# spaceml-org/STARCOP

Measured on AMD Instinct MI355X. Metric: 512x512 hyperspectral tiles/sec (train fwd+bwd), higher is better.
Workload: dtype f32; 1 GPU; configs[1]: HyperSTARCOP U-Net (smp.Unet mobilenet_v2, 4ch mag1c+RGB) train step fwd+loss+bwd+Adam, 512x512 tiles, fp32 HIP kernels (3x3 convs: fp32 operands split exactly into 16-bit terms on the matrix cores, fp32 accumulation; see config.precision and DESIGN.md section 2); batch_per_gpu=16, global_batch=16, parallelism=dp1, hipgraph=False, precision=fp32

## Files before the change

include/starcop_hip.h:

```cpp
#ifndef STARCOP_HIP_H
#define STARCOP_HIP_H

#include <stddef.h>
#include <stdint.h>

#ifdef __cplusplus
extern "C" {
#endif

typedef void* sc_stream;

enum sc_status {
  SC_OK = 0,
  SC_ERR_ARG = -1,
  SC_ERR_LAUNCH = -2,
  SC_ERR_NOTPD = -3,
  SC_ERR_NODEV = -4
};

enum sc_src_mode {
  SC_SRC_RAW = 0,
  SC_SRC_AFFINE = 1,
  SC_SRC_BNBWD = 2,
  SC_SRC_NORM = 3
// ... 69 lines not shown
size_t sc_packed_weight_floats_bx3(int Cout, int Cin, int co_t, int transpose_flip, int terms);
int sc_conv3x3_bx3(const sc_conv_args* a, sc_stream stream);

typedef struct sc_wgrad_args {
  sc_src dy;
  sc_src src[2];
  int32_t nsrc;
  int32_t N, H, W, Cout, Cin, ks;
  float* part; size_t part_floats;
  float* dw;
  int32_t terms;
  const float* absmax;
  const float* xbound[2];
} sc_wgrad_args;
size_t sc_wgrad_workspace_floats(int N, int H, int W, int Cout, int Cin, int ks);
int sc_conv2d_wgrad_mfma(const sc_wgrad_args* a, sc_stream stream);
typedef struct sc_wgrad_pending {
  const float* part; float* dw;
  int32_t nparts, taps, Cout, Cin, CoP, CiP;
  uint64_t total;
} sc_wgrad_pending;
int sc_conv2d_wgrad_mfma_deferred(const sc_wgrad_args* a, sc_wgrad_pending* pending_host, sc_stream stream);
int sc_wgrad_reduce_batch(const sc_wgrad_pending* descs_dev, const uint32_t* block_starts_dev, int n, uint32_t total_blocks,
                          sc_stream stream);
#define SC_PACK_THIN16 5
#define SC_PACK_PW3 6
size_t sc_packed_weight_floats_thin16(int Cout, int Cin, int transpose_flip);
int sc_pack_weights_thin16(const float* w_oihw, float* wpk, int Cout, int Cin, int transpose_flip, sc_stream stream);
int sc_conv3x3_thin16(const sc_conv_args* a, sc_stream stream);

#define SC_PACK_SP 7
size_t sc_packed_weight_floats_sp(int Cout, int Cup, int Cskip);
int sc_pack_weights_sp(const float* w_oihw, float* wpk, int Cout, int Cup, int Cskip, int terms, sc_stream stream);
int sc_sp_stat_rows(int N, int H, int W, int Cout);
int sc_conv3x3_sp(const sc_conv_args* a, sc_stream stream);
#define SC_PACK_SPD 8
size_t sc_packed_weight_floats_spd(int Cout, int Cup, int Cskip_tiles );
int sc_spd_vskip_ok(int Cup, int Cskip);
int sc_pack_weights_spd(const float* w_oihw, float* wpk, int Cout, int CinTotal, int Cup, int vskip, int terms, sc_stream stream);
int sc_conv3x3_sp_dgrad(const sc_conv_args* a, sc_stream stream);
size_t sc_sp_wgrad_workspace_bytes(int N, int H, int W, int Cout, int Cup);
int sc_conv3x3_sp_wgrad(const sc_wgrad_args* a, void* ws, size_t ws_bytes, sc_stream stream);
int sc_wgrad_scatter_cols(const float* src, float* dw, int Cout, int Ccols, int CinTotal, int col_off, sc_stream stream);

size_t sc_wgrad_thin16_workspace_floats(int N, int H, int W, int Cout, int Cin);
int sc_conv3x3_wgrad_thin16(const sc_wgrad_args* a, sc_stream stream);

size_t sc_packed_weight_floats_pw3(int Cout, int Cin, int transpose_flip);
int sc_conv1x1_pw3(const sc_conv_args* a, sc_stream stream);
int sc_conv1x1_pw3_variant(int N, int H, int W, int Cout);
size_t sc_wgrad_pw3_workspace_floats(int N, int H, int W, int Cout, int Cin);
int sc_conv1x1_wgrad_pw3(const sc_wgrad_args* a, sc_wgrad_pending* pending_host, sc_stream stream);
int sc_wgrad_pw3_variant(int N, int H, int W, int Cout, int Cin);

typedef struct sc_irb_args {
  sc_src x;
  const float* wpk_expand;
  const float* cst_expand;
  const float* w_dw;
  const float* cst_dw;
  const float* wpk_project;
  const float* cst_project;
  float* out;
  float* z_absmax;
  int32_t N, Cin, hidden, Cout, H, W, stride, residual;
} sc_irb_args;
int sc_irb_supported(int Cin, int hidden, int Cout, int H, int W, int stride);
int sc_irb_variant(int Cin, int hidden, int Cout, int stride);
int sc_irb_eval(const sc_irb_args* a, sc_stream stream);

typedef struct sc_irt_args {
  sc_src x;
  const float* w_expand;
  const float* w_dw;
  const float* cst_expand;
  int32_t N, Cin, hidden, H, W, stride;
} sc_irt_args;
int sc_irt_supported(int Cin, int hidden, int H, int W, int stride);
int sc_irt_rows(int stage, int N, int H, int W, int stride);
int sc_irt_bwd_rows(int N, int hidden, int H, int W);
size_t sc_irt_bwd_workspace_floats(int N, int Cin, int hidden, int H, int W);
int sc_irt_expand_stats(const sc_irt_args* a, float* stats , sc_stream stream);
int sc_irt_fwd(const sc_irt_args* a, float* d_out , float* stats_d , sc_stream stream);
int sc_irt_bwd(const sc_irt_args* a, const sc_src* dy_d, double* e_sums , double* dw_acc ,
               float* work, sc_stream stream);
int sc_irt_xmoments(const sc_irt_args* a, float* work, sc_stream stream);
int sc_irt_bwd_fix(const sc_irt_args* a, const float* cst_bwd_expand, float* work, float* dx, const float* add0, int accum,
                   sc_stream stream);
int sc_irt_wgrad_finalize(const sc_irt_args* a, const float* cst_bwd_expand, float* work, float* dw_expand, sc_stream stream);

size_t sc_wgrad_bx3_workspace_floats(int N, int H, int W, int Cout, int Cin);
int sc_conv3x3_wgrad_bx3(const sc_wgrad_args* a, sc_stream stream);

int sc_dwconv3x3_fwd(const sc_src* in, const float* w , float* out,
                     int N, int C, int Hin, int Win, int stride, float* stats ,
                     sc_stream stream);
typedef struct sc_bn_tail {
  const float* gamma; const float* beta;
  float* running_mean; float* running_var;
  float momentum, eps;
  float* cst;
  float* act_bound;
  uint32_t* tickets;
} sc_bn_tail;
int sc_dwconv3x3_fwd_bn(const sc_src* in, const float* w, float* out, int N, int C, int Hin, int Win, int stride, float* stats,
                        const sc_bn_tail* bn, sc_stream stream);
// ... 351 lines not shown
```

starcop_amd/_lib.py:

```python
import ctypes as C
import os
import subprocess

import torch

_HERE = os.path.dirname(os.path.abspath(__file__))
LIB_PATH = os.path.join(_HERE, "libstarcop_hip.so")
CSRC = os.path.join(_HERE, "csrc")

SC_CST = 8
STAT_CONV3, STAT_CONV1, STAT_DW, STAT_STEM, STAT_BNBWD, STAT_CONV1K, STAT_PW3 = 0, 1, 2, 3, 4, 5, 6

SRC_RAW, SRC_AFFINE, SRC_BNBWD, SRC_NORM = 0, 1, 2, 3
ACT_NONE, ACT_RELU, ACT_RELU6 = 0, 1, 2


class StarcopHipError(RuntimeError):
    pass


class sc_src(C.Structure):
    _fields_ = [("x", C.c_void_p), ("aux", C.c_void_p), ("cst", C.c_void_p),
                ("C", C.c_int32), ("mode", C.c_int32), ("act", C.c_int32), ("up", C.c_int32)]

# ... 210 lines not shown
    "sc_valid_mask_ne": (_i, [_vp, _i, _i, _i, _i, _d, C.c_int64, _vp, _vp]),
    "sc_mag1c_layout_columns": (_i, [_vp, _i, _i, _vp, _i, _i, _i, _vp, _vp, _vp, _vp, _vp, _vp, _vp]),
    "sc_mag1c_layout_ids_workspace_ints": (_sz, [C.c_int64, _i]),
    "sc_mag1c_layout_ids": (_i, [_vp, _vp, C.c_int64, _i, _i, _i, _vp, _vp, _vp, _vp, _vp, _vp, _vp, _vp]),
    "sc_trimmed_sum_workspace_bytes": (_sz, [_i]),
    "sc_trimmed_sums": (_i, [_vp, _i, _sz, _d, _vp, _vp, _sz, _vp]),
    "sc_band_ratio": (_i, [_vp, _vp, _vp, _i, _sz, _vp, _vp, _f, _f, _vp]),
    "sc_clip_scale": (_i, [_vp, _vp, _sz, _f, _f, _f, _f, _i, _vp]),
    "sc_mlr_workspace_bytes": (_sz, [_i, _sz, _i]),
    "sc_mlr_moments": (_i, [C.POINTER(sc_mlr_args), _vp, _sz, _vp]),
    "sc_mlr_solve": (_i, [C.POINTER(sc_mlr_args), _vp, _vp, _sz, _vp]),
    "sc_mlr_fit": (_i, [C.POINTER(sc_mlr_args), _vp, _vp, _sz, _vp]),
    "sc_mlr_predict": (_i, [C.POINTER(sc_mlr_args), _vp, _vp, _vp]),
    "sc_mlr_ratio": (_i, [C.POINTER(sc_mlr_args), _vp, _vp, _i, _i, _vp, _vp, _sz, _vp]),
    "sc_label_workspace_bytes": (_sz, [_i, _i, _i]),
    "sc_srf_bands": (_i, [C.POINTER(sc_srf_args), _vp]),
    "sc_window_stats_workspace_bytes": (_sz, [_i]),
    "sc_window_stats": (_i, [C.POINTER(sc_winstats_args), _vp, _sz, _vp]),
    "sc_glt_ortho": (_i, [C.POINTER(sc_ortho_args), _vp]),
    "sc_window_cut": (_i, [C.POINTER(sc_wcut_args), _vp]),
    "sc_scene_gather": (_i, [C.POINTER(sc_scene_args), _vp]),
    "sc_head_conv_fwd_k_mosaic": (_i, [C.POINTER(sc_src), _vp, _vp, _vp, _i, _i, C.c_int64, _vp, _vp, _i, _i, _i, _i, _i, _vp]),
    "sc_connected_components": (_i, [_vp, _i, _vp, _vp, _vp, _sz, _i, _i, _i, _vp]),
    "sc_proposed_mask": (_i, [_vp, C.c_int64, _vp, C.c_int64, _f, _i, _vp, _vp, _sz, _i, _i, _i, _vp]),
    "sc_packed_weight_floats_thin16": (_sz, [_i, _i, _i]),
    "sc_pack_weights_thin16": (_i, [_vp, _vp, _i, _i, _i, _vp]),
    "sc_conv3x3_thin16": (_i, [C.POINTER(sc_conv_args), _vp]),
    "sc_packed_weight_floats_sp": (_sz, [_i, _i, _i]),
    "sc_pack_weights_sp": (_i, [_vp, _vp, _i, _i, _i, _i, _vp]),
    "sc_sp_stat_rows": (_i, [_i, _i, _i, _i]),
    "sc_conv3x3_sp": (_i, [C.POINTER(sc_conv_args), _vp]),
    "sc_packed_weight_floats_spd": (_sz, [_i, _i, _i]),
    "sc_pack_weights_spd": (_i, [_vp, _vp, _i, _i, _i, _i, _i, _vp]),
    "sc_spd_vskip_ok": (_i, [_i, _i]),
    "sc_conv3x3_sp_dgrad": (_i, [C.POINTER(sc_conv_args), _vp]),
    "sc_sp_wgrad_workspace_bytes": (_sz, [_i, _i, _i, _i, _i]),
    "sc_conv3x3_sp_wgrad": (_i, [C.POINTER(sc_wgrad_args), _vp, _sz, _vp]),
    "sc_wgrad_scatter_cols": (_i, [_vp, _vp, _i, _i, _i, _i, _vp]),
    "sc_binary_opening": (_i, [_vp, _f, _i, _vp, _vp, _i, _i, _i, _vp]),
    "sc_threshold_confusion": (_i, [_vp, _vp, _vp, _vp, _i, _i, _vp, _vp, _i, _i, _i, _vp]),
    "sc_gather_augment": (_i, [_vp, _i, _i, _i, _i, _vp, _vp, _vp, _vp, _vp, _vp, _i, _i, _i, _i, _vp, _vp]),
    "sc_tile_window_sums": (_i, [_vp, _i, _i, _i, _vp, _vp, _i, _vp, _vp]),
    "sc_dwconv3x3_bwd_fused": (_i, [C.POINTER(sc_src), C.POINTER(sc_src), _vp, _vp, _vp, _vp, _i, _i, _i, _i, _i, _vp]),
    "sc_wgrad_thin16_workspace_floats": (_sz, [_i, _i, _i, _i, _i]),
    "sc_conv3x3_wgrad_thin16": (_i, [C.POINTER(sc_wgrad_args), _vp]),
    "sc_conv2d_wgrad_mfma_deferred": (_i, [C.POINTER(sc_wgrad_args), C.POINTER(sc_wgrad_pending), _vp]),
    "sc_wgrad_reduce_batch": (_i, [_vp, _vp, _i, C.c_uint32, _vp]),
    "sc_packed_weight_floats_pw3": (_sz, [_i, _i, _i]),
    "sc_conv1x1_pw3": (_i, [C.POINTER(sc_conv_args), _vp]),
    "sc_conv1x1_pw3_variant": (_i, [_i, _i, _i, _i]),
    "sc_wgrad_pw3_workspace_floats": (_sz, [_i, _i, _i, _i, _i]),
    "sc_wgrad_pw3_variant": (_i, [_i, _i, _i, _i, _i]),
    "sc_conv1x1_wgrad_pw3": (_i, [C.POINTER(sc_wgrad_args), C.POINTER(sc_wgrad_pending), _vp]),
    "sc_irb_supported": (_i, [_i, _i, _i, _i, _i, _i]),
    "sc_irb_variant": (_i, [_i, _i, _i, _i]),
    "sc_irb_eval": (_i, [C.POINTER(sc_irb_args), _vp]),
    "sc_irt_supported": (_i, [_i, _i, _i, _i, _i]),
    "sc_irt_rows": (_i, [_i, _i, _i, _i, _i]),
    "sc_irt_bwd_rows": (_i, [_i, _i, _i, _i]),
    "sc_irt_bwd_workspace_floats": (_sz, [_i, _i, _i, _i, _i]),
    "sc_irt_expand_stats": (_i, [C.POINTER(sc_irt_args), _vp, _vp]),
    "sc_irt_fwd": (_i, [C.POINTER(sc_irt_args), _vp, _vp, _vp]),
    "sc_irt_bwd": (_i, [C.POINTER(sc_irt_args), C.POINTER(sc_src), _vp, _vp, _vp, _vp]),
    "sc_irt_xmoments": (_i, [C.POINTER(sc_irt_args), _vp, _vp]),
    "sc_irt_bwd_fix": (_i, [C.POINTER(sc_irt_args), _vp, _vp, _vp, _vp, _i, _vp]),
    "sc_irt_wgrad_finalize": (_i, [C.POINTER(sc_irt_args), _vp, _vp, _vp, _vp]),
    "sc_maxpool2x2": (_i, [C.POINTER(sc_src), _vp, _i, _i, _i, _i, _vp]),
    "sc_upsample_bilinear2x": (_i, [C.POINTER(sc_src), _vp, _i, _i, _i, _i, _vp]),
    "sc_maxpool2x2_bwd": (_i, [C.POINTER(sc_src), _vp, _vp, _i, _i, _i, _i, _i, _vp]),
    "sc_upsample_bilinear2x_bwd": (_i, [_vp, _vp, _i, _i, _i, _i, _vp]),
    "sc_pwreg_param_floats": (_sz, [_i, _i, _i, _i]),
    "sc_pwreg_fwd": (_i, [_vp, _vp, _i, _i, _i, _i, _i, _i, _i, _vp, _vp]),
    "sc_reg_loss": (_i, [_vp, _vp, _sz, _i, _vp, _vp, _vp, _vp]),
    "sc_pwreg_sweep_blocks": (_i, [_i, _i, _i]),
    "sc_pwreg_train_sweep": (_i, [_vp, _vp, _vp, _i, _i, _i, _i, _i, _i, _i, _i, _vp, _vp]),
    "sc_pwreg_finalize": (_i, [_vp, _i, _vp, _i, _i, _i, _i, _d, _vp, _vp, _vp]),
    "sc_panel_minmax": (_i, [_vp, C.POINTER(sc_panel), _i, _vp, _vp]),
    "sc_render_panels": (_i, [_vp, C.POINTER(sc_panel), _i, _vp, _vp, _i, _i, _vp]),
    "sc_component_stats_workspace_bytes": (_sz, [_i, _i, _i, _i, _i]),
    "sc_component_stats": (_i, [C.POINTER(sc_cstats_args), _vp, _sz, _vp]),
    "sc_tiff_lzw_decode": (_i, [_vp, _sz, _vp, _sz, C.POINTER(C.c_size_t)]),
    "sc_tiff_unpredict": (_i, [_vp, _i, _i, _i, _i, _i, _i, _vp]),
}
REG_L1, REG_MSE, PWREG_G_FROM_MEMORY = 0, 1, 2
PWREG_MAXC, PWREG_PART_DOUBLES, REG_LOSS_PARTS = 16, 273, 256
PACK_SPD = 8
PACK_SP = 7
PACK_PW3 = 6
PACK_THIN16 = 5
TERMS_F16X2 = 4
SE_CROSS = 0xBA

_lib = None


def build(force=False):
    if force:
        subprocess.run(["make", "-C", CSRC, "clean"], check=True, stdout=subprocess.DEVNULL)
    r = subprocess.run(["make", "-C", CSRC, "-j", "4"], capture_output=True, text=True)
    if r.returncode != 0:
        raise StarcopHipError("building libstarcop_hip.so failed:\n" + r.stdout[-4000:] + r.stderr[-4000:])
    return LIB_PATH


def load():
    global _lib
# ... 76 lines not shown
```

starcop_amd/network.py:

```python
import ctypes as C
import math
import os

import torch
import torch.nn as nn

from . import _lib
from ._lib import (ACT_NONE, ACT_RELU, ACT_RELU6, SC_CST, sc_irb_args, sc_irt_args, SRC_AFFINE, SRC_BNBWD, SRC_NORM, SRC_RAW, STAT_BNBWD, sc_wgrad_pending,
                   PACK_PW3, PACK_SP, PACK_SPD, PACK_THIN16, STAT_PW3, STAT_CONV1, STAT_CONV1K, STAT_CONV3, STAT_DW, STAT_STEM, TERMS_F16X2, check, make_src, ptr, sc_bn_tail, sc_bnr_args,
                   sc_conv_args, sc_wgrad_args, stream)

MBV2_SETTINGS = ((1, 16, 1, 1), (6, 24, 2, 2), (6, 32, 3, 2), (6, 64, 4, 2),
                 (6, 96, 3, 1), (6, 160, 3, 2), (6, 320, 1, 1))
DECODER_CHANNELS = (256, 128, 64, 32, 16)
BN_EPS, BN_MOMENTUM = 1e-5, 0.1


def _conv_bn_act(cin, cout, k, stride=1, groups=1, act="relu6"):
    return nn.Sequential(nn.Conv2d(cin, cout, k, stride, (k - 1) // 2, groups=groups, bias=False),
                         nn.BatchNorm2d(cout, eps=BN_EPS, momentum=BN_MOMENTUM),
                         nn.ReLU6() if act == "relu6" else nn.ReLU())


class _InvertedResidual(nn.Module):
# ... 38 lines not shown
        cskips = (96, 32, 24, 16, 0)
        self.blocks = nn.ModuleList(_DecoderBlock(i, s, o) for i, s, o in zip(cins, cskips, DECODER_CHANNELS))


class _T:
    __slots__ = ("name", "C", "shift", "kind", "bn", "act", "buf", "grad", "cst", "cstb", "stats", "bsums",
                 "grad_written", "alias_grad_of", "res_grad")

    def __init__(self, name, Cn, shift, kind, bn=None, act=ACT_NONE):
        self.name, self.C, self.shift, self.kind, self.bn, self.act = name, Cn, shift, kind, bn, act
        self.buf = self.grad = self.cst = self.cstb = self.stats = self.bsums = None
        self.grad_written = False
        self.alias_grad_of = None
        self.res_grad = None


_BN_PRE = True
_COT_RATIO = 1.15
_COT_RATIO3 = 1.15
_HEAD_FUSED_BWD = True


def _pick_cot(M, ks=1):
    if M <= 16 and ks == 3:
        return 16
    if M <= 32:
        return 32
    p32, p64 = -(-M // 32) * 32, -(-M // 64) * 64
    return 64 if p64 <= p32 * (_COT_RATIO3 if ks == 3 else _COT_RATIO) else 32


_PW3 = os.environ.get("STARCOP_PW3", "1")
_PWS64 = os.environ.get("STARCOP_PWS64", "1") == "1"


def _use_pw3(which, N, HW, Cin, Cout):
    if _PW3 == "0" or (which == 2 and HW % 8):
        return False
    if _PW3 == "all":
        return True
    NP = N * HW
    npb = -(-NP // 32)
    if _PWS64 and HW == 4096 and which in (0, 1):
        K_, M_ = (Cin, Cout) if which == 0 else (Cout, Cin)
        if K_ in (16, 24, 32) and M_ <= 192 and (which == 1 or K_ in (24, 32)):
            return False
    if which == 0:
        return HW <= 4096 and (Cin <= 320 or npb * (-(-Cout // 32)) >= 1024)
    if which == 1:
        K, MB = Cout, -(-Cin // 32)
        return (K <= 192 and HW <= 4096 and NP <= 131072) or (K > 192 and HW <= 1024 and npb * MB >= 2048)
    KM = Cin * Cout
    return HW <= 1024 and NP <= 32768 and KM <= 300000 and (HW <= 256 or KM <= 32768)


_IRT = os.environ.get("STARCOP_IRT", "1")


def _use_irt(N, Cin, Hd, Hin, Win, stride):
    if _IRT == "0" or not _lib.load().sc_irt_supported(Cin, Hd, Hin, Win, stride):
        return False
    return _IRT == "all" or (Hin * Win >= 65536 and 4 * N * Hd * Hin * Win >= (256 << 20))


_IRB = os.environ.get("STARCOP_IRB", "1")


def _use_irb(N, Cin, hidden, Cout, H, W, stride):
    if _IRB == "0" or not _lib.load().sc_irb_supported(Cin, hidden, Cout, H, W, stride):
        return False
    if _IRB == "all":
        return True
    if stride == 2:
        return Cin <= 64 and hidden % 64 == 0 and H * W <= 25600
    return Cin <= 96 and hidden % 64 == 0 and Cout <= 128 and H * W <= 6400


_SP = os.environ.get("STARCOP_SP", "1")
_BNR = os.environ.get("STARCOP_BNR", "0") == "1"
_BNR_THIN = os.environ.get("STARCOP_BNR_THIN", "0") == "1"
_THIN_SPD = os.environ.get("STARCOP_THIN_SPD", "1") == "1"
_PACK_SIDE = os.environ.get("STARCOP_PACK_SIDE", "1") == "1"
_DW_TAIL_ROWS = int(os.environ.get("STARCOP_DW_TAIL_ROWS", "0"))
_SP_SKIPTILES = os.environ.get("STARCOP_SP_SKIPTILES", "1") == "1"


def _experiment(name, default=""):
    v = os.environ.get(name, default)
    if v not in ("", "0"):
        if os.environ.get("STARCOP_EXPERIMENT_OK") != "1":
            raise RuntimeError(f"{name}={v} is an elimination experiment (wrong results by design); set STARCOP_EXPERIMENT_OK=1 to run it")
        import warnings
        warnings.warn(f"starcop_amd: elimination experiment {name}={v} is ACTIVE -- results of this process are wrong by design")
    return v


_EXP_NO_WGRAD = _experiment("STARCOP_EXP_NO_WGRAD", "0") == "1"
_EXP_NO_BNFIN = _experiment("STARCOP_EXP_NO_BNFIN", "")
_EXP_SIDE2 = _experiment("STARCOP_EXP_SIDE2", "0") == "1"


_SP_TERMS = (TERMS_F16X2, 1)


def _use_sp(N, Ho, Wo, Cout):
    if _SP == "0" or Ho % 2 or Wo % 2:
# ... 363 lines not shown
            n_dw = 0
            irt_e = {self._ops[i]["out"].name for i in plan.irt}
            plan.irt_esums, plan.irt_work = {}, {}
            for i_e in plan.irt:
                cv, tin, te = self._ops[i_e]["conv"], self._ops[i_e]["ins"][0], self._ops[i_e]["out"]
                Hi, Wi = H >> tin.shift, W >> tin.shift
                plan.irt_esums[te.name] = torch.empty(lib.sc_irt_bwd_rows(N, cv.out_channels, Hi, Wi) * cv.out_channels * 2, dtype=torch.float64, device=dev)
                plan.irt_work[te.name] = torch.empty(lib.sc_irt_bwd_workspace_floats(N, cv.in_channels, cv.out_channels, Hi, Wi), **f32)
            for op in self._ops:
                o = op["out"]
                Ho, Wo = H >> o.shift, W >> o.shift
                if op["type"] != "head" and o.kind != "fin" and o.name not in irt_e:
                    plan.grad[o.name] = torch.empty((N, o.C, Ho, Wo), **f32)
                if op["type"] == "add":
                    plan.grad[o.name] = torch.empty((N, o.C, Ho, Wo), **f32)
                conv = op.get("conv")
                if op["type"] in ("pw", "conv3"):
                    ws = max(ws, lib.sc_wgrad_workspace_floats(N, Ho, Wo, conv.out_channels, conv.in_channels,
                                                               conv.kernel_size[0]))
                    if conv.kernel_size[0] == 3:
                        ws = max(ws, lib.sc_wgrad_bx3_workspace_floats(N, Ho, Wo, conv.out_channels, conv.in_channels))
                        if conv.out_channels <= 16 and conv.in_channels in (16, 32):
                            ws = max(ws, lib.sc_wgrad_thin16_workspace_floats(N, Ho, Wo, conv.out_channels, conv.in_channels))
                    if op.get("up"):
                        up = max(up, N * op["ins"][0].C * Ho * Wo)
                elif op["type"] == "stem":
                    ws = max(ws, lib.sc_stem_wgrad_workspace_floats(N, conv.in_channels, H, W))
                elif op["type"] == "head":
                    ws = max(ws, lib.sc_head_wgrad_workspace_floats(N, conv.in_channels, Ho, Wo))
                elif op["type"] == "dw":
                    n_dw += conv.out_channels * 9
            spw_b, spw_sk = 0, 0
            for op in self._ops:
                if op["type"] == "conv3" and op.get("up"):
                    cv, o_ = op["conv"], op["out"]
                    Hq, Wq = H >> o_.shift, W >> o_.shift
                    cu_ = op["ins"][0].C
                    if _use_spw(N, Hq, Wq, cv.out_channels, cu_):
                        spw_b = max(spw_b, lib.sc_sp_wgrad_workspace_bytes(N, Hq, Wq, cv.out_channels, cu_))
                        if cv.in_channels > cu_:
                            spw_sk = max(spw_sk, cv.out_channels * (cv.in_channels - cu_) * 9)
                            ws = max(ws, lib.sc_wgrad_bx3_workspace_floats(N, Hq, Wq, cv.out_channels, cv.in_channels - cu_),
                                     lib.sc_wgrad_workspace_floats(N, Hq, Wq, cv.out_channels, cv.in_channels - cu_, 3))
            plan.spw_ws = torch.empty(spw_b + 256, dtype=torch.uint8, device=dev) if spw_b else None
            plan.spw_skip = torch.empty(spw_sk, **f32) if spw_sk else None
            plan.ws = torch.empty(ws, **f32)
            plan.ws_floats = ws
            plan.pw_part, plan.pw_table = {}, None
            if self.batch_pw_reduce:
                for i, op in enumerate(self._ops):
                    if op["type"] == "pw" and i not in plan.irt:
                        conv, o = op["conv"], op["out"]
                        Hq, Wq = H >> o.shift, W >> o.shift
                        nfl = (lib.sc_wgrad_pw3_workspace_floats(N, Hq, Wq, conv.out_channels, conv.in_channels)
                               if _use_pw3(2, N, Hq * Wq, conv.in_channels, conv.out_channels)
                               else lib.sc_wgrad_workspace_floats(N, Hq, Wq, conv.out_channels, conv.in_channels, 1))
                        plan.pw_part[i] = torch.empty(nfl, **f32)
            plan.up_tmp = torch.empty(max(up, 1), **f32)
            plan.dw_acc = torch.zeros(n_dw, dtype=torch.float64, device=dev)
            plan.gmax = torch.zeros(len(self._ops) + 1, dtype=torch.float32, device=dev)
            for t in self._tensors.values():
                if t.bn is not None:
                    plan.bsums_v[t.name] = torch.empty(plan.brows[t.name] * t.C * 2, dtype=torch.float64, device=dev)
            plan.dwrows, plan.dwsums = {}, {}
            for op in self._ops:
                if op["type"] == "dw" and op["ins"][0].bn is not None and op["ins"][0].name not in irt_e:
                    ti = op["ins"][0]
                    plan.dwrows[ti.name] = lib.sc_stat_rows(STAT_DW, N, H >> ti.shift, W >> ti.shift)
                    plan.dwsums[ti.name] = torch.empty(plan.dwrows[ti.name] * ti.C * 2, dtype=torch.float64, device=dev)
            plan.dlogits = torch.empty((N, 1, H, W), **f32)
            plan.has_grad = True
        return plan

    def _pack_all(self, need_bwd):
        lib = _lib.load()
        ver = (tuple(p._version for p in self.parameters()), self._terms, self.split_bf16, self.thin16)
        pv = self._pack_version
        need_irb = (not need_bwd) and bool(getattr(self, "_irb_layers", None))
        if pv is not None and pv[0] == ver and (pv[1] or not need_bwd) and (pv[2] or not need_irb):
            return
        st = stream()
        dev = self._pflat.device
        if not hasattr(self, "_wpk"):
            self._wpk = {}
        for i, op in enumerate(self._ops):
            if op["type"] not in ("pw", "conv3"):
                continue
            conv = op["conv"]
            co, ci, ks = conv.out_channels, conv.in_channels, conv.kernel_size[0]
            ent = self._wpk.get(i)
            tf_, tb_ = self._terms
            if ent is None or ent["f"].device != dev or ent["split"] != (self.split_bf16, tf_, tb_):
                cf, cb = _pick_cot(co, ks), _pick_cot(ci, ks)
                if ks == 3 and co <= 16 and ci >= 32 and self.split_bf16:
                    cf = 32
                xf = self.split_bf16 and ks == 3 and cf >= 32
                xb = self.split_bf16 and ks == 3 and cb >= 32
                nf = lib.sc_packed_weight_floats_bx3(co, ci, cf, 0, tf_) if xf else lib.sc_packed_weight_floats(co, ci, ks, cf, 0)
                nb = lib.sc_packed_weight_floats_bx3(co, ci, cb, 1, tb_) if xb else lib.sc_packed_weight_floats(co, ci, ks, cb, 1)
                ent = dict(cot_f=cf, cot_b=cb, bx3_f=xf, bx3_b=xb, split=(self.split_bf16, tf_, tb_), terms_f=tf_, terms_b=tb_,
                           f=torch.empty(nf, dtype=torch.float32, device=dev),
                           b=torch.empty(nb, dtype=torch.float32, device=dev), tf=None, tb=None, tsd=None)
                if self.split_bf16 and self.thin16 and ks == 3 and len(op["ins"]) == 1:
                    if tf_ == TERMS_F16X2 and co <= 16 and ci in (16, 32):
                        ent["tf"] = torch.empty(lib.sc_packed_weight_floats_thin16(co, ci, 0), dtype=torch.float32, device=dev)
                    if tb_ == TERMS_F16X2 and ci <= 16 and co in (16, 32):
                        ent["tb"] = torch.empty(lib.sc_packed_weight_floats_thin16(co, ci, 1), dtype=torch.float32, device=dev)
# ... 706 lines not shown
            wa.dw = gv(conv.weight).data_ptr()
            wa.terms = self._terms[1]
            wa.absmax = gmax_slot.get(o.name)
            if ty == "conv3":
                for k_, t_ in enumerate(ins):
                    wa.xbound[k_] = self._xbound(plan, t_)
            flop = 2.0 * N * Ho * Wo * conv.out_channels * conv.in_channels * ks * ks
            if (op.get("up") and plan.spw_ws is not None and self.split_bf16 and self._terms[1] == TERMS_F16X2
                    and _use_spw(N, Ho, Wo, conv.out_channels, ins[0].C)):
                cu_ = ins[0].C
                wu = sc_wgrad_args()
                wu.dy, wu.nsrc = dy, 1
                wu.src[0] = wa.src[0]
                wu.N, wu.H, wu.W, wu.Cout, wu.Cin, wu.ks = N, Ho, Wo, o.C, conv.in_channels, 3
                wu.part, wu.part_floats, wu.dw = None, 0, gv(conv.weight).data_ptr()
                wu.terms, wu.absmax = self._terms[1], gmax_slot.get(o.name)
                wu.xbound[0] = self._xbound(plan, ins[0])
                wsb = C.c_void_p((plan.spw_ws.data_ptr() + 255) & ~255)
                nb = plan.spw_ws.numel() - 256
                tok = self._pb("k_wgrad3_bx3 (+reduce)", flop, 0.0, 2.0 * N * (Ho // 2) * (Wo // 2) * 9 * conv.out_channels * cu_
                               + 2.0 * N * Ho * Wo * 9 * conv.out_channels * (conv.in_channels - cu_))
                wgrad_launch(lambda sx, wu=wu, wsb=wsb, nb=nb: check(lib.sc_conv3x3_sp_wgrad(C.byref(wu), wsb, nb, sx)))
                if len(ins) == 2:
                    csk_ = ins[1].C
                    wk = sc_wgrad_args()
                    wk.dy, wk.nsrc = dy, 1
                    wk.src[0] = wa.src[1]
                    wk.N, wk.H, wk.W, wk.Cout, wk.Cin, wk.ks = N, Ho, Wo, o.C, csk_, 3
                    wk.part, wk.part_floats, wk.dw = plan.ws.data_ptr(), plan.ws_floats, plan.spw_skip.data_ptr()
                    wk.terms, wk.absmax = self._terms[1], gmax_slot.get(o.name)
                    wk.xbound[0] = self._xbound(plan, ins[1])
                    wsk = lib.sc_conv3x3_wgrad_bx3 if (o.C >= 32 and csk_ >= 32) else lib.sc_conv2d_wgrad_mfma

                    def skip_cols(sx, wk=wk, wsk=wsk, csk_=csk_, cu_=cu_, conv=conv, o=o):
                        check(wsk(C.byref(wk), sx))
                        check(lib.sc_wgrad_scatter_cols(ptr(plan.spw_skip), ptr(gv(conv.weight)), o.C, csk_, conv.in_channels, cu_, sx))
                    wgrad_launch(skip_cols)
                self._pe(tok)
                wfn = None
            else:
                wfn = (lib.sc_conv3x3_wgrad_bx3 if (self.split_bf16 and ks == 3 and conv.out_channels >= 32 and conv.in_channels >= 32)
                       else lib.sc_conv2d_wgrad_mfma)
            if (wfn is not None and self.split_bf16 and self.thin16 and ks == 3 and self._terms[1] == TERMS_F16X2 and len(ins) == 1
                    and conv.out_channels <= 16 and conv.in_channels in (16, 32) and Wo % 2 == 0):
                wfn = lib.sc_conv3x3_wgrad_thin16
            tok = None if wfn is None else self._pb(
                "k_wgrad3_bx3 (+reduce)" if wfn is lib.sc_conv3x3_wgrad_bx3 else
                "k_wgrad_thin_h (+reduce)" if wfn is lib.sc_conv3x3_wgrad_thin16 else f"k_wgrad_mfma<{ks}> (+reduce)", flop)
            if wfn is None:
                pass
            elif ty == "pw" and i in plan.pw_part:
                wa.part = plan.pw_part[i].data_ptr(); wa.part_floats = plan.pw_part[i].numel()
                pend = sc_wgrad_pending()
                wdef = (lib.sc_conv1x1_wgrad_pw3 if _use_pw3(2, N, Ho * Wo, conv.in_channels, conv.out_channels)
                        else lib.sc_conv2d_wgrad_mfma_deferred)
                wgrad_launch(lambda sx, wa=wa, pend=pend, wdef=wdef: check(wdef(C.byref(wa), C.byref(pend), sx)), second=True)
                pw_pending.append(pend)
                if i == last_pw:
                    reduce_pointwise_batch()
            else:
                wgrad_launch(lambda sx, wfn=wfn, wa=wa: check(wfn(C.byref(wa), sx)))
            self._pe(tok)
            if ins[0].kind == "input":
                continue
            ent = self._wpk[i]
            a = sc_conv_args()
            a.nsrc = 1
            a.src[0] = dy
            a.wpk = ent["b"].data_ptr()
            a.N, a.H, a.W, a.Cout = N, Ho, Wo, conv.in_channels
            a.ks, a.co_t = ks, ent["cot_b"]
            a.terms = ent["terms_b"]
            a.absmax = gmax_slot.get(o.name)
            if ent["bx3_b"]:
                conv_dgrad = lib.sc_conv3x3_bx3
            elif ty == "pw" and _use_pw3(1, N, Ho * Wo, conv.in_channels, conv.out_channels):
                conv_dgrad = lib.sc_conv1x1_pw3
                a.wpk = ent["pb"].data_ptr()
            elif _use_ksplit(N, Ho * Wo, conv.out_channels, conv.in_channels, ks):
                conv_dgrad = lib.sc_conv1x1_ksplit
            else:
                conv_dgrad = lib.sc_conv2d_mfma
            a.add0 = None; a.add1 = None; a.stats = None
            a.accum0 = a.accum1 = 0
            bx3_plain = ent["bx3_b"] and not (a.terms == TERMS_F16X2 and (conv.out_channels + 15) // 16 >= 16 and conv.out_channels <= 256)
            gin_elems = N * conv.in_channels * Ho * Wo
            if op.get("up") and ent["bx3_b"]:
                gin_elems -= N * ins[0].C * Ho * Wo * 3 // 4
            thin_b = (ent["tb"] is not None and not op.get("up") and ins[0].name not in written and res_of.get(ins[0].name) is None)
            thin_sd = (ent.get("tsd") is not None and op.get("up") and len(ins) == 1 and a.terms == TERMS_F16X2 and _THIN_SPD and not _BNR
                       and Ho % 2 == 0 and Wo % 2 == 0)
            fle = None
            if (op.get("up") and ent.get("spd") is not None and ent["terms_b"] in _SP_TERMS and self.split_bf16
                    and _use_spd(N, Ho, Wo, ins[0].C, conv.in_channels - ins[0].C)):
                cu_ = ins[0].C
                fle = (2.0 * N * (Ho // 2) * (Wo // 2) * 16 * conv.out_channels * (-(-cu_ // 128) * 128 + (128 * -(-(conv.in_channels - cu_) // 32) if ent["spd_stiles"] else 0))
                       + (0.0 if (ent["spd_vskip"] or ent["spd_stiles"]) else 2.0 * N * Ho * Wo * 9 * conv.out_channels * (conv.in_channels - cu_)))
            tok = self._pb("k_conv3_thin_h (fwd+dgrad)" if (thin_b or thin_sd) else
                           self._bx3_family("dgrad") if ent["bx3_b"] else f"k_conv_mfma<{ks}> (fwd+dgrad)", flop,
                           4.0 * (2 * N * o.C * Ho * Wo + gin_elems + conv.weight.numel()), fle)
            if (op.get("up") and ent.get("spd") is not None and ent["terms_b"] in _SP_TERMS and self.split_bf16
                    and _use_spd(N, Ho, Wo, ins[0].C, conv.in_channels - ins[0].C)):
                if ent["spd_vskip"] or ent["spd_stiles"]:
                    t_up, t_sk = ins
                    a.Cout, a.csplit = conv.in_channels, t_up.C
                    a.wpk = ent["spd"].data_ptr()
                    a.out0, a.out1 = plan.grad[t_up.name].data_ptr(), plan.grad[t_sk.name].data_ptr()
# ... 170 lines not shown
```

Baseline: 1447 tiles/s.

## Add narrow-side pointwise wgrad kernel with shared-memory reuse for deep layers

Adds a new 1x1 conv weight-gradient kernel for layers where one channel side is at most 160. The narrow operand is converted and split into 16-bit terms once per workgroup, then shared through LDS across four waves that each own 32 wide-side channels. Loads are double-buffered in registers, and partial sums are reduced afterwards by the existing deferred batch reduce. It is selected only for specific deep-layer shapes (HW 1024 or 256 at N=16 with a wide side above a threshold). The cost is a new code path plus partial-sum workspace.

```diff
diff --git a/include/starcop_hip.h b/include/starcop_hip.h
--- a/include/starcop_hip.h
+++ b/include/starcop_hip.h
@@ -145,6 +145,10 @@
 size_t sc_wgrad_pw3_workspace_floats(int N, int H, int W, int Cout, int Cin);
 int sc_conv1x1_wgrad_pw3(const sc_wgrad_args* a, sc_wgrad_pending* pending_host, sc_stream stream);
 int sc_wgrad_pw3_variant(int N, int H, int W, int Cout, int Cin);
+int sc_wgrad_pwn_supported(int N, int H, int W, int Cout, int Cin);
+int sc_wgrad_pwn_variant(int N, int H, int W, int Cout, int Cin);
+size_t sc_wgrad_pwn_workspace_floats(int N, int H, int W, int Cout, int Cin);
+int sc_conv1x1_wgrad_pwn(const sc_wgrad_args* a, sc_wgrad_pending* pending_host, sc_stream stream);
 
 typedef struct sc_irb_args {
   sc_src x;
diff --git a/starcop_amd/_lib.py b/starcop_amd/_lib.py
--- a/starcop_amd/_lib.py
+++ b/starcop_amd/_lib.py
@@ -286,6 +286,10 @@
     "sc_wgrad_pw3_workspace_floats": (_sz, [_i, _i, _i, _i, _i]),
     "sc_wgrad_pw3_variant": (_i, [_i, _i, _i, _i, _i]),
     "sc_conv1x1_wgrad_pw3": (_i, [C.POINTER(sc_wgrad_args), C.POINTER(sc_wgrad_pending), _vp]),
+    "sc_wgrad_pwn_supported": (_i, [_i, _i, _i, _i, _i]),
+    "sc_wgrad_pwn_variant": (_i, [_i, _i, _i, _i, _i]),
+    "sc_wgrad_pwn_workspace_floats": (_sz, [_i, _i, _i, _i, _i]),
+    "sc_conv1x1_wgrad_pwn": (_i, [C.POINTER(sc_wgrad_args), C.POINTER(sc_wgrad_pending), _vp]),
     "sc_irb_supported": (_i, [_i, _i, _i, _i, _i, _i]),
     "sc_irb_variant": (_i, [_i, _i, _i, _i]),
     "sc_irb_eval": (_i, [C.POINTER(sc_irb_args), _vp]),
diff --git a/starcop_amd/csrc/conv_pwn.hip b/starcop_amd/csrc/conv_pwn.hip
--- /dev/null
+++ b/starcop_amd/csrc/conv_pwn.hip
@@ -0,0 +1,285 @@
+#include "sc_split.h"
+
+namespace {
+
+struct PwnP {
+  SrcD dy, s;
+  int NP, HW, Cout, Cin;
+  int ksteps;
+  int per_wg;
+  int CoP, CiP;
+  int WB;
+  float* part;
+};
+
+struct PwnCst { float c[5]; };
+
+template <bool ISDY>
+__device__ __forceinline__ PwnCst pwn_cst(const float* cst, unsigned ch) {
+  PwnCst k;
+  if (ISDY) {
+    const float4 c0 = *reinterpret_cast<const float4*>(cst + (size_t)ch * SC_CST);
+    k.c[0] = c0.x; k.c[1] = c0.y; k.c[2] = c0.z; k.c[3] = c0.w; k.c[4] = cst[(size_t)ch * SC_CST + 4];
+  } else {
+    const float2 c0 = *reinterpret_cast<const float2*>(cst + (size_t)ch * SC_CST);
+    k.c[0] = c0.x; k.c[1] = c0.y; k.c[2] = k.c[3] = k.c[4] = 0.f;
+  }
+  return k;
+}
+
+template <bool ISDY, bool BNB>
+__device__ __forceinline__ void pwn_convert(const float4 (&g)[2], const float4 (&y)[2], const PwnCst& k, bool ok, float lo, float hi,
+                                            uintx4 (&t)[3]) {
+  const float g8[8] = {g[0].x, g[0].y, g[0].z, g[0].w, g[1].x, g[1].y, g[1].z, g[1].w};
+  float v[8];
+  if (ISDY && BNB) {
+    const float y8[8] = {y[0].x, y[0].y, y[0].z, y[0].w, y[1].x, y[1].y, y[1].z, y[1].w};
+#pragma unroll
+    for (int j = 0; j < 8; ++j) {
+      const float r = sc_pro_bnbwd(g8[j], y8[j], k.c[0], k.c[1], k.c[2], k.c[3], k.c[4], lo, hi);
+      v[j] = ok ? r : 0.f;
+    }
+  } else {
+#pragma unroll
+    for (int j = 0; j < 8; ++j) {
+      const float r = sc_pro_affine(g8[j], k.c[0], k.c[1], lo, hi);
+      v[j] = ok ? r : 0.f;
+    }
+  }
+  split8(v, t);
+}
+
+template <int NB, int TW, bool DYW, bool BNB>
+__global__ __launch_bounds__(256, 2) void k_pwn_wgrad(const PwnP p) {
+  static_assert(NB >= 1 && NB <= 5 && TW >= 1 && TW <= 2 && NB * TW * 16 <= 160, "at most 160 accumulator registers per lane");
+  constexpr int NJ = (NB + 3) / 4;
+  constexpr int PD = 2;
+  __shared__ uintx4 s_n[2][NB][3][64];
+  const int tid = threadIdx.x, lane = tid & 63, wave = __builtin_amdgcn_readfirstlane(tid >> 6);
+  const int l31 = lane & 31, lhi = lane >> 5;
+  const int HW = p.HW;
+  const SrcD& ws = DYW ? p.dy : p.s;
+  const SrcD& ns = DYW ? p.s : p.dy;
+  const int Cw = DYW ? p.Cout : p.Cin, Cn = DYW ? p.Cin : p.Cout;
+  const float wlo = sc_act_lo(ws.act), whi = sc_act_hi(ws.act);
+  const float nlo = sc_act_lo(ns.act), nhi = sc_act_hi(ns.act);
+  const int wb0 = (blockIdx.y * 4 + wave) * TW;
+  const bool wlive = wb0 < p.WB;
+  PwnCst w_k[TW]; bool w_ok[TW]; size_t w_o[TW];
+#pragma unroll
+  for (int t = 0; t < TW; ++t) {
+    const int ch = (wb0 + t) * 32 + l31;
+    w_ok[t] = ch < Cw;
+    const unsigned c = w_ok[t] ? ch : 0;
+    w_k[t] = pwn_cst<DYW>(ws.cst, c);
+    w_o[t] = (size_t)c * HW;
+  }
+  PwnCst n_k[NJ]; bool n_ok[NJ]; size_t n_o[NJ];
+#pragma unroll
+  for (int j = 0; j < NJ; ++j) {
+    const int ch = (wave + 4 * j) * 32 + l31;
+    n_ok[j] = wave + 4 * j < NB && ch < Cn;
+    const unsigned c = n_ok[j] ? ch : 0;
+    n_k[j] = pwn_cst<!DYW>(ns.cst, c);
+    n_o[j] = (size_t)c * HW;
+  }
+
+  floatx16 acc[TW][NB];
+#pragma unroll
+  for (int t = 0; t < TW; ++t)
+#pragma unroll
+    for (int q = 0; q < NB; ++q)
+#pragma unroll
+      for (int r = 0; r < 16; ++r) acc[t][q][r] = 0.f;
+
+  const int k_begin = blockIdx.x * p.per_wg;
+  const int k_end = min(k_begin + p.per_wg, p.ksteps);
+  float4 wg[PD][TW][2], wy[PD][TW][2], ng[PD][NJ][2], ny[PD][NJ][2];
+  bool live[PD];
+
+#define PWN_ISSUE(slot, kst_)                                                                           \
+  {                                                                                                     \
+    const int kq_ = (kst_);                                                                             \
+    const int g0_ = (kq_ * 2 + lhi) * 8;                                                                \
+    live[slot] = kq_ < k_end && g0_ < p.NP;                                                             \
+    const int gc_ = live[slot] ? g0_ : 0;                                                               \
+    const int n_ = gc_ / HW;                                                                            \
+    const size_t px_ = (size_t)(gc_ - n_ * HW);                                                         \
+    const size_t wbase_ = (size_t)n_ * Cw * HW + px_, nbase_ = (size_t)n_ * Cn * HW + px_;              \
+    if (wlive) {                                                                                        \
+      _Pragma("unroll") for (int t = 0; t < TW; ++t) {                                                  \
+        const size_t o_ = wbase_ + w_o[t];                                                              \
+        wg[slot][t][0] = *reinterpret_cast<const float4*>(ws.x + o_);                                   \
+        wg[slot][t][1] = *reinterpret_cast<const float4*>(ws.x + o_ + 4);                               \
+        if (DYW && BNB) {                                                                               \
+          wy[slot][t][0] = *reinterpret_cast<const float4*>(ws.aux + o_);                               \
+          wy[slot][t][1] = *reinterpret_cast<const float4*>(ws.aux + o_ + 4);                           \
+        }                                                                                               \
+      }                                                                                                 \
+    }                                                                                                   \
+    _Pragma("unroll") for (int j = 0; j < NJ; ++j) {                                                    \
+      if (wave + 4 * j < NB) {                                                                          \
+        const size_t o_ = nbase_ + n_o[j];                                                              \
+        ng[slot][j][0] = *reinterpret_cast<const float4*>(ns.x + o_);                                   \
+        ng[slot][j][1] = *reinterpret_cast<const float4*>(ns.x + o_ + 4);                               \
+        if (!DYW && BNB) {                                                                              \
+          ny[slot][j][0] = *reinterpret_cast<const float4*>(ns.aux + o_);                               \
+          ny[slot][j][1] = *reinterpret_cast<const float4*>(ns.aux + o_ + 4);                           \
+        }                                                                                               \
+      }                                                                                                 \
+    }                                                                                                   \
+  }
+
+#pragma unroll
+  for (int s = 0; s < PD; ++s) {
+#pragma unroll
+    for (int t = 0; t < TW; ++t) { wy[s][t][0] = wy[s][t][1] = make_float4(0.f, 0.f, 0.f, 0.f); }
+#pragma unroll
+    for (int j = 0; j < NJ; ++j) { ny[s][j][0] = ny[s][j][1] = make_float4(0.f, 0.f, 0.f, 0.f); }
+  }
+#pragma unroll
+  for (int s = 0; s < PD; ++s) PWN_ISSUE(s, k_begin + s)
+
+  for (int k0 = k_begin; k0 < k_end; k0 += PD) {
+#pragma unroll
+    for (int s = 0; s < PD; ++s) {
+      const int k = k0 + s;
+      if (k >= k_end) break;
+      const int buf = s & 1;
+#pragma unroll
+      for (int j = 0; j < NJ; ++j) {
+        if (wave + 4 * j < NB) {
+          uintx4 t3[3];
+          pwn_convert<!DYW, BNB>(ng[s][j], ny[s][j], n_k[j], live[s] && n_ok[j], nlo, nhi, t3);
+#pragma unroll
+          for (int q = 0; q < 3; ++q) s_n[buf][wave + 4 * j][q][lane] = t3[q];
+        }
+      }
+      uintx4 a[TW][3];
+      if (wlive) {
+#pragma unroll
+        for (int t = 0; t < TW; ++t) pwn_convert<DYW, BNB>(wg[s][t], wy[s][t], w_k[t], live[s] && w_ok[t], wlo, whi, a[t]);
+      }
+      PWN_ISSUE(s, k + PD)
+      __syncthreads();
+      if (wlive) {
+#pragma unroll
+        for (int q = 0; q < NB; ++q) {
+          uintx4 b[3];
+#pragma unroll
+          for (int u = 0; u < 3; ++u) b[u] = s_n[buf][q][u][lane];
+#pragma unroll
+          for (int t = 0; t < TW; ++t) acc[t][q] = DYW ? mfma6(a[t], b, acc[t][q]) : mfma6(b, a[t], acc[t][q]);
+        }
+      }
+    }
+  }
+#undef PWN_ISSUE
+
+  float* part = p.part + (size_t)blockIdx.x * p.CoP * p.CiP;
+#pragma unroll
+  for (int t = 0; t < TW; ++t) {
+    if (wb0 + t >= p.WB) continue;
+#pragma unroll
+    for (int q = 0; q < NB; ++q)
+#pragma unroll
+      for (int r = 0; r < 16; ++r) {
+        const int row = 8 * (r >> 2) + 4 * lhi + (r & 3);
+        const int co = (DYW ? wb0 + t : q) * 32 + row;
+        const int ci = (DYW ? q : wb0 + t) * 32 + l31;
+        part[(size_t)co * p.CiP + ci] = acc[t][q][r];
+      }
+  }
+}
+
+constexpr int PWN_MAX_NARROW = 160;
+
+struct PwnPlan { int ok, nb, tw, dyw, WB, cols, per_wg, nparts, CoP, CiP, ksteps; };
+
+PwnPlan plan_pwn(int N, int H, int W, int Cout, int Cin) {
+  PwnPlan pl{};
+  if (N <= 0 || H <= 0 || W <= 0 || Cout <= 0 || Cin <= 0) return pl;
+  const long HW = (long)H * W, NP = (long)N * HW;
+  if (HW % 8 != 0 || NP > (1L << 30) || HW > (1L << 30)) return pl;
+  pl.dyw = Cout >= Cin;
+  const int Cw = pl.dyw ? Cout : Cin, Cn = pl.dyw ? Cin : Cout;
+  if (Cn > PWN_MAX_NARROW) return pl;
+  pl.ok = 1;
+  pl.nb = (Cn + 31) / 32;
+  pl.WB = (Cw + 31) / 32;
+  pl.tw = 1;
+  pl.cols = (pl.WB + 4 * pl.tw - 1) / (4 * pl.tw);
+  pl.CoP = (Cout + 31) / 32 * 32;
+  pl.CiP = (Cin + 31) / 32 * 32;
+  pl.ksteps = (int)((NP + 15) / 16);
+  int want = 512 / pl.cols;
+  if (want < 1) want = 1;
+  int per_wg = (pl.ksteps + want - 1) / want;
+  if (per_wg < 8) per_wg = 8;
+  pl.per_wg = per_wg;
+  pl.nparts = (pl.ksteps + per_wg - 1) / per_wg;
+  return pl;
+}
+
+template <int NB, int TW, bool DYW>
+void pwn_launch(dim3 grid, hipStream_t st, const PwnP& p) {
+  if (p.dy.mode == SC_SRC_BNBWD) hipLaunchKernelGGL((k_pwn_wgrad<NB, TW, DYW, true>), grid, dim3(256), 0, st, p);
+  else hipLaunchKernelGGL((k_pwn_wgrad<NB, TW, DYW, false>), grid, dim3(256), 0, st, p);
+}
+
+}
+
+extern "C" int sc_wgrad_pwn_supported(int N, int H, int W, int Cout, int Cin) { return plan_pwn(N, H, W, Cout, Cin).ok; }
+
+extern "C" int sc_wgrad_pwn_variant(int N, int H, int W, int Cout, int Cin) {
+  const PwnPlan pl = plan_pwn(N, H, W, Cout, Cin);
+  return pl.ok ? 100 * pl.dyw + 10 * pl.nb + pl.tw : -1;
+}
+
+extern "C" size_t sc_wgrad_pwn_workspace_floats(int N, int H, int W, int Cout, int Cin) {
+  const PwnPlan pl = plan_pwn(N, H, W, Cout, Cin);
+  if (!pl.ok) return 0;
+  const size_t E = (size_t)pl.CoP * pl.CiP;
+  return (size_t)pl.nparts * E + sc_reduce_scratch_floats(pl.nparts, E);
+}
+
+extern "C" int sc_conv1x1_wgrad_pwn(const sc_wgrad_args* a, sc_wgrad_pending* pending, sc_stream stream) {
+  SC_REQUIRE(a != nullptr, "sc_conv1x1_wgrad_pwn: null args");
+  SC_REQUIRE(a->ks == 1 && a->nsrc == 1, "sc_conv1x1_wgrad_pwn: ks must be 1 with a single source");
+  SC_REQUIRE(a->src[0].C == a->Cin && a->dy.C == a->Cout, "sc_conv1x1_wgrad_pwn: channel mismatch");
+  SC_REQUIRE(a->dy.up == 0 && a->src[0].up == 0, "sc_conv1x1_wgrad_pwn: sources cannot be upsampled");
+  SC_REQUIRE(a->src[0].mode == SC_SRC_RAW || a->src[0].mode == SC_SRC_AFFINE, "sc_conv1x1_wgrad_pwn: input must be a RAW or AFFINE source");
+  SC_REQUIRE(a->dy.mode != SC_SRC_NORM && (a->dy.mode != SC_SRC_BNBWD || a->dy.aux), "sc_conv1x1_wgrad_pwn: bad dy source");
+  SC_REQUIRE(a->dy.x && a->src[0].x && a->part && a->dw, "sc_conv1x1_wgrad_pwn: null tensor");
+  const PwnPlan pl = plan_pwn(a->N, a->H, a->W, a->Cout, a->Cin);
+  SC_REQUIRE(pl.ok, "sc_conv1x1_wgrad_pwn: unsupported shape (N %d, %d x %d, %d <- %d channels: H*W %% 8 == 0, narrow side <= %d)",
+             a->N, a->H, a->W, a->Cout, a->Cin, PWN_MAX_NARROW);
+  const size_t need = sc_wgrad_pwn_workspace_floats(a->N, a->H, a->W, a->Cout, a->Cin);
+  SC_REQUIRE(a->part_floats >= need, "sc_conv1x1_wgrad_pwn: workspace too small (%zu < %zu floats)", a->part_floats, need);
+  PwnP p;
+  p.dy = to_srcd(a->dy); p.s = to_srcd(a->src[0]);
+  if (p.dy.mode == SC_SRC_RAW) { p.dy.cst = sc_identity_cst_table(p.dy.C); p.dy.act = SC_ACT_NONE; SC_REQUIRE(p.dy.cst, "sc_conv1x1_wgrad_pwn: identity constants unavailable"); }
+  if (p.s.mode == SC_SRC_RAW) { p.s.cst = sc_identity_cst_table(p.s.C); p.s.act = SC_ACT_NONE; SC_REQUIRE(p.s.cst, "sc_conv1x1_wgrad_pwn: identity constants unavailable"); }
+  SC_REQUIRE(p.dy.cst && p.s.cst, "sc_conv1x1_wgrad_pwn: source constants missing");
+  p.NP = a->N * a->H * a->W; p.HW = a->H * a->W; p.Cout = a->Cout; p.Cin = a->Cin;
+  p.ksteps = pl.ksteps; p.per_wg = pl.per_wg; p.CoP = pl.CoP; p.CiP = pl.CiP; p.WB = pl.WB; p.part = a->part;
+  const dim3 grid(pl.nparts, pl.cols);
+  hipStream_t st = (hipStream_t)stream;
+  const int variant = sc_wgrad_pwn_variant(a->N, a->H, a->W, a->Cout, a->Cin);
+  switch (variant) {
+#define SC_PWN(NB, TW)                                          \
+    case 100 + 10 * NB + TW: pwn_launch<NB, TW, true>(grid, st, p); break; \
+    case 10 * NB + TW: pwn_launch<NB, TW, false>(grid, st, p); break;
+    SC_PWN(1, 1) SC_PWN(2, 1) SC_PWN(3, 1) SC_PWN(4, 1) SC_PWN(5, 1)
+#undef SC_PWN
+    default: sc_set_error("sc_conv1x1_wgrad_pwn: bad shape"); return SC_ERR_ARG;
+  }
+  SC_LAUNCH_OK("sc_conv1x1_wgrad_pwn");
+  if (pending) {
+    pending->part = a->part; pending->dw = a->dw; pending->nparts = pl.nparts; pending->taps = 1;
+    pending->Cout = a->Cout; pending->Cin = a->Cin; pending->CoP = pl.CoP; pending->CiP = pl.CiP;
+    pending->total = (uint64_t)a->Cout * a->Cin;
+    return SC_OK;
+  }
+  return sc_wgrad_finish(a->part, pl.nparts, 1, a->Cout, a->Cin, pl.CoP, pl.CiP, a->dw, st);
+}
diff --git a/starcop_amd/network.py b/starcop_amd/network.py
--- a/starcop_amd/network.py
+++ b/starcop_amd/network.py
@@ -114,6 +114,19 @@
         return (K <= 192 and HW <= 4096 and NP <= 131072) or (K > 192 and HW <= 1024 and npb * MB >= 2048)
     KM = Cin * Cout
     return HW <= 1024 and NP <= 32768 and KM <= 300000 and (HW <= 256 or KM <= 32768)
+
+
+_PWN = os.environ.get("STARCOP_PWN", "1")
+_PWN_RULE = {1024: (16384, 384), 256: (4096, 960)}
+
+
+def _use_pwn(N, HW, Cin, Cout):
+    if _PWN == "0" or not _lib.load().sc_wgrad_pwn_supported(N, 1, HW, Cout, Cin):
+        return False
+    if _PWN == "all":
+        return True
+    NP_, wide = _PWN_RULE.get(HW, (0, 0))
+    return NP_ == N * HW and max(Cin, Cout) >= wide
 
 
 _IRT = os.environ.get("STARCOP_IRT", "1")
@@ -583,7 +596,9 @@
                     if op["type"] == "pw" and i not in plan.irt:
                         conv, o = op["conv"], op["out"]
                         Hq, Wq = H >> o.shift, W >> o.shift
-                        nfl = (lib.sc_wgrad_pw3_workspace_floats(N, Hq, Wq, conv.out_channels, conv.in_channels)
+                        nfl = (lib.sc_wgrad_pwn_workspace_floats(N, Hq, Wq, conv.out_channels, conv.in_channels)
+                               if _use_pwn(N, Hq * Wq, conv.in_channels, conv.out_channels)
+                               else lib.sc_wgrad_pw3_workspace_floats(N, Hq, Wq, conv.out_channels, conv.in_channels)
                                if _use_pw3(2, N, Hq * Wq, conv.in_channels, conv.out_channels)
                                else lib.sc_wgrad_workspace_floats(N, Hq, Wq, conv.out_channels, conv.in_channels, 1))
                         plan.pw_part[i] = torch.empty(nfl, **f32)
@@ -1396,7 +1411,8 @@
             elif ty == "pw" and i in plan.pw_part:
                 wa.part = plan.pw_part[i].data_ptr(); wa.part_floats = plan.pw_part[i].numel()
                 pend = sc_wgrad_pending()
-                wdef = (lib.sc_conv1x1_wgrad_pw3 if _use_pw3(2, N, Ho * Wo, conv.in_channels, conv.out_channels)
+                wdef = (lib.sc_conv1x1_wgrad_pwn if _use_pwn(N, Ho * Wo, conv.in_channels, conv.out_channels)
+                        else lib.sc_conv1x1_wgrad_pw3 if _use_pw3(2, N, Ho * Wo, conv.in_channels, conv.out_channels)
                         else lib.sc_conv2d_wgrad_mfma_deferred)
                 wgrad_launch(lambda sx, wa=wa, pend=pend, wdef=wdef: check(wdef(C.byref(wa), C.byref(pend), sx)), second=True)
                 pw_pending.append(pend)
```

Result: no change. 1454 tiles/s, median of 4 (+0.5%).
